# yuliangguo/OmniFusion

Hardware: AMD Instinct MI355X
Metric: panoramas/sec at 512x1024 ERP, N=18 256^2 patches; equi2pers+pers2equi GB/s vs HBM peak (higher is better)
Workload: dtype f16x3 (fp16 hi/lo pairs, fp32 accumulate: fp32-class); 1 GPU; cfg2/cfg4 shard: 8 panoramas/GPU/step, 512x1024 ERP, fov 80, nrows 4 (18 patches); full single-pass spherical_fusion forward (confidence=True) at patch size 128 — the only size the reference network exists at (SURVEY 0.1); random-init weights (seed 42); inputs resident in HBM; resample pair at 18x256^2 reported in roofline_resample; per_gpu_batch=8, global_batch=8, parallelism=image-sharded x1, execution=3 forwards in flight per GPU on 3 streams (spherical_fusion.pipelined)

## Files before the change

omnifusion_amd/csrc/omni_conv_sh.hip:

```cpp
#include "omni_conv_sh_common.h"

namespace {

__constant__ float wino_coef[16][4] = {
    {1, 0, 0, 0}, {1, 1, 0, 0}, {1, -1, 0, 0}, {0, -1, 0, 0},
    {1, 0, 1, 0}, {1, 1, 1, 1}, {1, -1, 1, -1}, {0, -1, 0, -1},
    {1, 0, -1, 0}, {1, 1, -1, -1}, {1, -1, -1, 1}, {0, -1, 0, 1},
    {0, 0, -1, 0}, {0, 0, -1, -1}, {0, 0, -1, 1}, {0, 0, 0, 1}};
template <int BM, int BN, int WM, int WN, int NST = 3, int NL = 0, bool PP = false, bool WINO = false, bool X1 = false>
__global__ __launch_bounds__(64 * (WM * WN + NL)) void conv_sh_kernel(ShConvArgs a)
{
    static_assert(!(WINO && X1), "Winograd: f16x3 only");
    static_assert(!PP || (NL > 0 && WM * WN == 8 && NST >= 3), "ping-pong: eight matrix waves (two per SIMD) + loader waves, three stages");
    static_assert(!WINO || (PP && BM / WM == 32 && BN / WN == 32), "Winograd: the ping-pong kernel with 32 x 32 wave tiles");
    constexpr int NW = WM * WN, LW = NL > 0 ? NL : NW, RPP = 8 * LW;
    constexpr int TM = BM / WM / 32, TN = BN / WN / 32;
    constexpr int APASS = BM / RPP, BPASS = BN / RPP, LPS = APASS + BPASS;
    static_assert(APASS >= 1 && BPASS >= 1, "a tile side must cover at least one DMA pass");
    constexpr int A_BYTES = BM * 128, STAGE = (BM + BN) * 128;
    __shared__ __attribute__((aligned(1024))) unsigned char lds[NST * STAGE];
    __shared__ long long cst[OMNI_ABL(32768) ? 256 : 1];
    const bool stamped = OMNI_ABL(32768) && blockIdx.x == 0 && blockIdx.y == 0 && a.ws != nullptr && a.splitk <= 1;
    auto cstamp = [&](int k) { if (OMNI_ABL(32768) && stamped && (threadIdx.x & 63) == 0 && k < 256) cst[k] = clock64(); };
    auto cdump = [&]() { if (OMNI_ABL(32768) && stamped && threadIdx.x == 0) for (int i = 0; i < 256; ++i) reinterpret_cast<long long*>(a.ws)[i] = cst[i]; };
// ... 477 lines not shown

template <bool X1, int BM, int BN, int WM, int WN, int NST = 3, int NL = 0>
void launch_sh(ShConvArgs a, hipStream_t s)
{
    const int tiles = ((a.rows + BM - 1) / BM) * (a.Cout / BN);
    if constexpr (NL > 0 && WM * WN == 8) {
        if (omni_options().conv_pingpong) {
            hipLaunchKernelGGL((conv_sh_kernel<BM, BN, WM, WN, NST, NL, true, false, X1>), dim3(tiles, a.splitk > 1 ? a.splitk : 1), dim3(64 * (WM * WN + NL)), 0, s, a);
            return;
        }
    }
    hipLaunchKernelGGL((conv_sh_kernel<BM, BN, WM, WN, NST, NL, false, false, X1>), dim3(tiles, a.splitk > 1 ? a.splitk : 1), dim3(64 * (WM * WN + NL)), 0, s, a);
}

}

static int conv2d_sh_impl(const void* src1, const void* src2, const void* wt16, const float* bias,
                          const void* res, void* dst, int fmt, int M, int H, int W, int C1, int C2, int Cout,
                          int KH, int KW, int stride, int pad, int act, int splitk, float* ws, size_t ws_bytes,
                          const float* post, size_t post_elems, omni_stream_t stream, bool reduce = true);
extern "C" int omni_conv2d_sh_f16x3_ws(const void* src1, const void* src2, const void* wt16, const float* bias,
                                       const void* res, void* dst, int fmt, int M, int H, int W, int C1, int C2, int Cout,
                                       int KH, int KW, int stride, int pad, int act, int splitk, float* ws, size_t ws_bytes,
                                       omni_stream_t stream)
{
    return conv2d_sh_impl(src1, src2, wt16, bias, res, dst, fmt, M, H, W, C1, C2, Cout, KH, KW, stride, pad, act, splitk, ws, ws_bytes,
                          nullptr, 0, stream);
}
extern "C" int omni_conv2d_sh_f16x3_post_ws(const void* src1, const void* src2, const void* wt16, const float* bias,
                                            const void* res, void* dst, int fmt, int M, int H, int W, int C1, int C2, int Cout,
                                            int KH, int KW, int stride, int pad, int act, int splitk, float* ws, size_t ws_bytes,
                                            const float* post, size_t post_elems, omni_stream_t stream)
{
    return conv2d_sh_impl(src1, src2, wt16, bias, res, dst, fmt, M, H, W, C1, C2, Cout, KH, KW, stride, pad, act, splitk, ws, ws_bytes,
                          post, post_elems, stream);
}
extern "C" int omni_gemm_sh_f16x3_ln512_ws(const void* x, const void* wt16, const float* bias, const float* res, float* tok, const float* ln_g, const float* ln_b,
                                           float eps, void* y, int fmt, int rows, int K, int splitk, float* ws, size_t ws_bytes, omni_stream_t stream)
{
    if (!x || !wt16 || !tok || !ln_g || !ln_b || !y) OMNI_FAIL(OMNI_ERR_INVALID, "omni_gemm_sh_f16x3_ln512: null pointer");
    if (rows <= 0 || K <= 0 || K % 32) OMNI_FAIL(OMNI_ERR_INVALID, "omni_gemm_sh_f16x3_ln512: bad shape");
    if (fmt & 8) OMNI_FAIL(OMNI_ERR_UNSUPPORTED, "omni_gemm_sh_f16x3_ln512: no f16x1 form (fmt bit 3)");
    const int S = std::min(splitk, K / 32);
    if (S < 2) OMNI_FAIL(OMNI_ERR_INVALID, "omni_gemm_sh_f16x3_ln512: needs a split-K plan (splitk >= 2); an unsplit GEMM writes its result in its own epilogue");
    const int rc = conv2d_sh_impl(x, nullptr, wt16, bias, res, tok, 2, rows, 1, 1, K, 0, 512, 1, 1, 1, 0, OMNI_ACT_NONE, S, ws, ws_bytes, nullptr, 0, stream, false);
    if (rc != OMNI_OK) return rc;
    hipStream_t s = (hipStream_t)stream;
    if (fmt & 1) hipLaunchKernelGGL(sh_splitk_reduce_ln512_kernel<true>, dim3((rows + 3) / 4), dim3(256), 0, s, (const float*)ws, bias, res, tok, ln_g, ln_b, y, rows, S, (size_t)rows * 512, eps);
    else         hipLaunchKernelGGL(sh_splitk_reduce_ln512_kernel<false>, dim3((rows + 3) / 4), dim3(256), 0, s, (const float*)ws, bias, res, tok, ln_g, ln_b, y, rows, S, (size_t)rows * 512, eps);
    OMNI_HIP(hipGetLastError());
    return OMNI_OK;
}

template <bool X1>
static void conv_sh_select(const ShConvArgs& a, int fmt, hipStream_t s)
{
    const int KH = a.KH, KW = a.KW, stride = a.stride, pad = a.pad, H = a.H, W = a.W, M = a.M, Cout = a.Cout;
    const int ksteps = KH * KW * ((a.C1 + a.C2) / 32);
    const long long rows = a.rows;
    if (a.splitk <= 1 && KH == 3 && KW == 3 && stride == 1 && pad == 1 && H == W && (W == 16 || (W == 8 && omni_options().conv_img >= 2)) && rows % 128 == 0 &&
        Cout % 64 == 0 && !(fmt & 4) && omni_options().conv_img > 0 && !omni_options().conv_nohalo) {
        const int grid = (int)(rows / 128) * (Cout / 64);
        if (omni_options().conv_halo_bn == 32) {
            if (W == 16) omni_halo_launch(&a, 32, 4, false, 16, X1, 2 * grid, s);
            else         omni_halo_launch(&a, 32, 4, false, 8, X1, 2 * grid, s);
        }
        else if (W == 16) omni_halo_launch(&a, 64, 4, false, 16, X1, grid, s);
        else         omni_halo_launch(&a, 64, 4, false, 8, X1, grid, s);
        return;
    }
    if (a.splitk <= 1 && KH == 3 && KW == 3 && stride == 1 && pad == 1 && W % HT_W == 0 && H % 4 == 0 && !omni_options().conv_nohalo) {
        const int th = (H % 8 == 0 && omni_options().conv_halo_th == 8) ? 8 : 4;
        const int grid = M * (H / th) * (W / HT_W);
        if (th == 8) {
            if (Cout % 64 == 0 && omni_options().conv_halo_bn != 32) omni_halo_launch(&a, 64, 8, false, 0, X1, grid * (Cout / 64), s);
            else                omni_halo_launch(&a, 32, 8, false, 0, X1, grid * (Cout / 32), s);
        } else {
            const bool bn32 = omni_options().conv_halo_bn == 32 || ((fmt & 4) && omni_options().conv_halo_bn_lat == 32);
            if (Cout % 64 == 0 && !bn32) omni_halo_launch(&a, 64, 4, false, 0, X1, grid * (Cout / 64), s);
            else                omni_halo_launch(&a, 32, 4, false, 0, X1, grid * (Cout / 32), s);
        }
        return;
    }
    int tile = omni_options().conv_sh_tile;
    if (tile < 0) tile = 8;
    const int pm = omni_options().conv_pm;
    const bool pm_shape = pm > 0 && KH == 3 && KW == 3 && stride == 1 && pad == 1 && H == W && (W == 8 || W == 4) && Cout % 64 == 0 && !a.post &&
                          omni_options().conv_pingpong && !(pm == 3 && W != 8) && !(pm == 4 && W != 4);
    if (pm_shape && pm == 2) { omni_conv_pm_launch(&a, Cout % 128 == 0 ? 128 : 64, X1, s); return; }
    const bool big256 = tile == 8 && Cout % 128 == 0 && ((rows + 255) / 256) * (long long)(Cout / 128) * a.splitk >= std::max(1, omni_options().conv_big_blocks);
    if (pm_shape && tile == 8 && !big256) {
        if (Cout % 128 == 0 && ((rows + 127) / 128) * (long long)(Cout / 128) * a.splitk >= 128) { omni_conv_pm_launch(&a, 128, X1, s); return; }
        if (((rows + 127) / 128) * (long long)(Cout / 64) * a.splitk >= 128) { omni_conv_pm_launch(&a, 64, X1, s); return; }
    }
    if (Cout % 64 != 0) launch_sh<X1, 128, 32, 4, 1>(a, s);
    else if (tile == 2 && Cout % 128 == 0) launch_sh<X1, 128, 128, 2, 2>(a, s);
    else if (tile == 1) launch_sh<X1, 128, 64, 2, 2>(a, s);
    else if (tile == 3) launch_sh<X1, 128, 64, 4, 2>(a, s);
    else if (tile == 4 && Cout % 128 == 0) launch_sh<X1, 128, 128, 4, 2>(a, s);
    else if (tile == 8 && Cout % 128 == 0 && ((rows + 255) / 256) * (long long)(Cout / 128) * a.splitk >= std::max(1, omni_options().conv_big_blocks)) launch_sh<X1, 256, 128, 4, 2>(a, s);
    else if (tile == 8 && Cout % 128 == 0 && ((rows + 127) / 128) * (long long)(Cout / 128) * a.splitk >= 128) launch_sh<X1, 128, 128, 4, 2, 3, 4>(a, s);
    else if (tile == 8 && ((rows + 127) / 128) * (long long)(Cout / 64) * a.splitk >= 128) launch_sh<X1, 128, 64, 4, 2, 3, 4>(a, s);
    else if (tile == 9 && Cout % 128 == 0 && ((rows + 255) / 256) * (long long)(Cout / 128) * a.splitk >= 128) launch_sh<X1, 256, 128, 4, 2>(a, s);
    else if (tile == 9 && Cout % 128 == 0 && ((rows + 127) / 128) * (long long)(Cout / 128) * a.splitk >= 128) launch_sh<X1, 128, 128, 4, 2>(a, s);
    else if (tile == 9 && ((rows + 127) / 128) * (long long)(Cout / 64) * a.splitk >= 128) launch_sh<X1, 128, 64, 4, 2>(a, s);
    else if (tile >= 5 && tile <= 7 && Cout % 128 == 0 && ((rows + 127) / 128) * (long long)(Cout / 128) * a.splitk >= (32ll << (tile - 4))) launch_sh<X1, 128, 128, 4, 2>(a, s);
    else if (tile >= 5 && tile <= 7 && ((rows + 127) / 128) * (long long)(Cout / 64) * a.splitk >= (32ll << (tile - 4))) launch_sh<X1, 128, 64, 4, 2>(a, s);
    else if (((rows + 63) / 64) * (long long)(Cout / 64) * a.splitk <= 256 && ksteps >= 8 && !omni_options().conv_nodeep) {
        if (omni_options().conv_deep_loaders) launch_sh<X1, 64, 64, 2, 2, 6, 4>(a, s);
        else launch_sh<X1, 64, 64, 2, 2, 6>(a, s);
    }
    else launch_sh<X1, 64, 64, 2, 2>(a, s);
// ... 22 lines not shown
    const long long rows = (long long)M * a.Ho * a.Wo;
    if (rows <= 0 || rows >= (1ll << 31) || (long long)M * H * W >= (1ll << 31))
        OMNI_FAIL(OMNI_ERR_UNSUPPORTED, "omni_conv2d_sh: too many pixels for 32-bit row indices");
    a.rows = (int)rows;
    const int ksteps = KH * KW * ((C1 + C2) / 32);
    if ((long long)M * H * W * (C1 > C2 ? C1 : C2) * 4 >= (1ll << 31) || (long long)Cout * ksteps * 128 >= (1ll << 31))
        OMNI_FAIL(OMNI_ERR_UNSUPPORTED, "omni_conv2d_sh: an operand of 2 GiB or more (32-bit buffer offsets)");
    int S = splitk;
    if (S > ksteps) S = ksteps;
    if (S > 1 && (!ws || ws_bytes < (size_t)S * rows * Cout * sizeof(float)))
        OMNI_FAIL(OMNI_ERR_INVALID, "omni_conv2d_sh: split-K workspace too small");
    a.splitk = S > 1 ? S : 1; a.ws = ws;
    a.wt_major = omni_options().conv_wt_major == 2 || (omni_options().conv_wt_major == 1 &&
                 (long long)Cout * ksteps * 128 > (long long)M * H * W * (C1 + C2) * 4) ? 1 : 0;
    a.post = post; a.post_rows = 1; a.wino_th = a.wino_tw = a.wino_pix = 0;
    if (post) {
        if (Cout <= 0 || post_elems == 0 || post_elems % (size_t)Cout || post_elems / (size_t)Cout > 0x7fffffffull)
            OMNI_FAIL(OMNI_ERR_INVALID, "omni_conv2d_sh: the post-activation addend must hold whole rows of Cout channels");
        if (a.splitk > 1) OMNI_FAIL(OMNI_ERR_UNSUPPORTED, "omni_conv2d_sh: no post-activation addend with split-K");
        a.post_rows = (unsigned)(post_elems / (size_t)Cout);
    }
    hipStream_t s = (hipStream_t)stream;
    if (fmt & 8) conv_sh_select<true>(a, fmt, s);
    else         conv_sh_select<false>(a, fmt, s);
    OMNI_HIP(hipGetLastError());
    if (a.splitk > 1 && reduce) {
        const size_t n4 = (size_t)rows * Cout / 4;
        hipLaunchKernelGGL(sh_splitk_reduce_kernel, dim3((unsigned)((n4 + 255) / 256)), dim3(256), 0, s, (const float*)ws, bias, res, dst,
                           n4, Cout, a.splitk, (size_t)rows * Cout, act, a.dst_sh, a.res_f32);
        OMNI_HIP(hipGetLastError());
    }
    return OMNI_OK;
}

extern "C" int omni_splitk_reduce_ln512(const float* parts, int nparts, const float* bias, const float* res, float* tok, const float* lg, const float* lb,
                                        float eps, void* y, int fmt, int rows, omni_stream_t stream)
{
    if (!parts || nparts < 1 || !tok || !lg || !lb || !y || rows <= 0) OMNI_FAIL(OMNI_ERR_INVALID, "omni_splitk_reduce_ln512: null pointer or empty input");
    hipStream_t s = (hipStream_t)stream;
    if (fmt & 1) hipLaunchKernelGGL(sh_splitk_reduce_ln512_kernel<true>, dim3((rows + 3) / 4), dim3(256), 0, s, parts, bias, res, tok, lg, lb, y, rows, nparts, (size_t)rows * 512, eps);
    else         hipLaunchKernelGGL(sh_splitk_reduce_ln512_kernel<false>, dim3((rows + 3) / 4), dim3(256), 0, s, parts, bias, res, tok, lg, lb, y, rows, nparts, (size_t)rows * 512, eps);
    OMNI_HIP(hipGetLastError());
    return OMNI_OK;
}

OMNI_SH_OVERFLOW_ACCESSOR(omni_sh_overflow_conv)

extern "C" int omni_sh_overflow(int* flag, int reset)
{
    if (!flag) OMNI_FAIL(OMNI_ERR_INVALID, "omni_sh_overflow: null output");
    OMNI_HIP(hipDeviceSynchronize());
    unsigned v = 0;
    if (omni_sh_overflow_conv(&v, reset) != 0 || omni_sh_overflow_halo(&v, reset) != 0 || omni_sh_overflow_up2(&v, reset) != 0 ||
        omni_sh_overflow_rows(&v, reset) != 0 || omni_sh_overflow_net(&v, reset) != 0 || omni_sh_overflow_pm(&v, reset) != 0)
        OMNI_FAIL(OMNI_ERR_HIP, "omni_sh_overflow: could not read the device flag");
    *flag = v ? 1 : 0;
    return OMNI_OK;
}

extern "C" int omni_sh_from_f32(const float* src, void* dst, size_t n, omni_stream_t stream)
{
    if (!src || !dst || n % 32) OMNI_FAIL(OMNI_ERR_INVALID, "omni_sh_from_f32: null pointer or n % 32 != 0");
    if (n == 0) return OMNI_OK;
    hipLaunchKernelGGL(sh_from_f32_kernel, dim3((unsigned)((n / 4 + 255) / 256)), dim3(256), 0, (hipStream_t)stream, src, dst, n / 4);
    OMNI_HIP(hipGetLastError());
    return OMNI_OK;
}
extern "C" int omni_sh_to_f32(const void* src, float* dst, size_t n, omni_stream_t stream)
{
    if (!src || !dst || n % 32) OMNI_FAIL(OMNI_ERR_INVALID, "omni_sh_to_f32: null pointer or n % 32 != 0");
    if (n == 0) return OMNI_OK;
    hipLaunchKernelGGL(sh_to_f32_kernel, dim3((unsigned)((n / 4 + 255) / 256)), dim3(256), 0, (hipStream_t)stream, src, dst, n / 4);
    OMNI_HIP(hipGetLastError());
    return OMNI_OK;
}

namespace {

__global__ __launch_bounds__(256) void wino_input_sh_kernel(const void* __restrict__ src, void* __restrict__ V, int M, int H, int W, int C, size_t nt)
{
    const size_t i = (size_t)blockIdx.x * 256 + threadIdx.x;
    const int cq = C >> 2;
    if (i >= nt * cq) return;
    const size_t tl = i / cq;
    const int c = (int)(i - tl * cq) * 4;
    const int tw = W >> 1, th = H >> 1;
    const int m = (int)(tl / (size_t)(th * tw)), rem = (int)(tl - (size_t)m * th * tw), ty = rem / tw, tx = rem - ty * tw;
    f4v d[4][4];
#pragma unroll
    for (int a_ = 0; a_ < 4; ++a_)
#pragma unroll
        for (int b_ = 0; b_ < 4; ++b_) {
            const int y = 2 * ty - 1 + a_, x = 2 * tx - 1 + b_;
            d[a_][b_] = ((unsigned)y < (unsigned)H && (unsigned)x < (unsigned)W) ? act_load4<true>(src, (((size_t)m * H + y) * W + x) * C + c) : (f4v)(0.0f);
        }
    f4v u[4][4];
#pragma unroll
    for (int b_ = 0; b_ < 4; ++b_) { u[0][b_] = d[0][b_] - d[2][b_]; u[1][b_] = d[1][b_] + d[2][b_]; u[2][b_] = d[2][b_] - d[1][b_]; u[3][b_] = d[1][b_] - d[3][b_]; }
#pragma unroll
    for (int xi = 0; xi < 4; ++xi) {
        const f4v v0 = u[xi][0] - u[xi][2], v1 = u[xi][1] + u[xi][2], v2 = u[xi][2] - u[xi][1], v3 = u[xi][1] - u[xi][3];
        act_store4<true>(V, ((size_t)(4 * xi + 0) * nt + tl) * C + c, v0);
        act_store4<true>(V, ((size_t)(4 * xi + 1) * nt + tl) * C + c, v1);
        act_store4<true>(V, ((size_t)(4 * xi + 2) * nt + tl) * C + c, v2);
        act_store4<true>(V, ((size_t)(4 * xi + 3) * nt + tl) * C + c, v3);
    }
}
// ... 43 lines not shown
```

omnifusion_amd/csrc/omni_conv_sh_common.h:

```cpp
#pragma once
#include <stdlib.h>
#include <algorithm>
#include <type_traits>
#include "omni_internal.h"
#include "omni_sh.h"

#ifndef OMNI_CONV_ABL
#define OMNI_CONV_ABL 0
#endif
#define OMNI_ABL(bit) ((OMNI_CONV_ABL & (bit)) != 0)
#ifndef OMNI_PP_PRIO
#define OMNI_PP_PRIO 0
#endif
#ifndef OMNI_G1_PW
#define OMNI_G1_PW 4
#endif

namespace {

typedef float f16v __attribute__((ext_vector_type(16)));
typedef float f4v __attribute__((ext_vector_type(4)));
typedef _Float16 h8v __attribute__((ext_vector_type(8)));
typedef _Float16 h4v __attribute__((ext_vector_type(4)));
typedef _Float16 h2v __attribute__((ext_vector_type(2)));
// ... 149 lines not shown
            if (a.res) {
#pragma unroll
                for (int e = 0; e < 4; ++e) { v0[e] += fmaf((float)rl[kk][e], 4.8828125e-4f, (float)rh[kk][e]); v1[e] += fmaf((float)rl[kk][4 + e], 4.8828125e-4f, (float)rh[kk][4 + e]); }
            }
            if (a.act == OMNI_ACT_RELU) {
#pragma unroll
                for (int e = 0; e < 4; ++e) { v0[e] = fmaxf(v0[e], 0.f); v1[e] = fmaxf(v1[e], 0.f); }
            } else if (a.act == OMNI_ACT_GELU) {
#pragma unroll
                for (int e = 0; e < 4; ++e) { v0[e] = 0.5f * v0[e] * (1.0f + erff(v0[e] * 0.70710678118654752440f)); v1[e] = 0.5f * v1[e] * (1.0f + erff(v1[e] * 0.70710678118654752440f)); }
            }
            if (post) { v0 += pa[kk]; v1 += pb[kk]; }
            h4v h0, l0, h1, l1;
            sh_split4(v0, h0, l0); sh_split4(v1, h1, l1);
            h8v oh, ol;
#pragma unroll
            for (int e = 0; e < 4; ++e) { oh[e] = h0[e]; oh[4 + e] = h1[e]; ol[e] = l0[e]; ol[4 + e] = l1[e]; }
            *reinterpret_cast<h8v*>((unsigned char*)a.dst + off[kk]) = oh;
            *reinterpret_cast<h8v*>((unsigned char*)a.dst + off[kk] + 64) = ol;
        }
    }
}

__device__ __forceinline__ void splitk_finish(f4v v, size_t o, const float* __restrict__ bias, const void* __restrict__ res, void* __restrict__ dst,
                                              int Cout, int act, int dst_sh, int res_f32)
{
    if (bias) v += *reinterpret_cast<const f4v*>(bias + (o % Cout));
    if (res && res_f32) v += *reinterpret_cast<const f4v*>((const float*)res + o);
    else if (res) {
        const unsigned char* rp = (const unsigned char*)res + sh_off(o);
        v += sh_join4(*reinterpret_cast<const h4v*>(rp), *reinterpret_cast<const h4v*>(rp + 64));
    }
    if (act == OMNI_ACT_RELU) { v.x = fmaxf(v.x, 0.f); v.y = fmaxf(v.y, 0.f); v.z = fmaxf(v.z, 0.f); v.w = fmaxf(v.w, 0.f); }
    else if (act == OMNI_ACT_GELU) {
#pragma unroll
        for (int e = 0; e < 4; ++e) v[e] = 0.5f * v[e] * (1.0f + erff(v[e] * 0.70710678118654752440f));
    }
    if (dst_sh) {
        h4v hi, lo; sh_split4(v, hi, lo);
        unsigned char* dp = (unsigned char*)dst + sh_off(o);
        *reinterpret_cast<h4v*>(dp) = hi; *reinterpret_cast<h4v*>(dp + 64) = lo;
    } else {
        *reinterpret_cast<f4v*>((float*)dst + o) = v;
    }
}

constexpr int HT_W = 32, HPW = HT_W + 2;

}

void omni_halo_launch(const void* args, int bn, int th, bool up2, int iw, bool x1, unsigned grid, hipStream_t s);
void omni_conv_pm_launch(const void* args, int bn, bool x1, hipStream_t s);
int omni_sh_overflow_pm(unsigned* out, int reset);
int omni_sh_overflow_halo(unsigned* out, int reset);
int omni_sh_overflow_up2(unsigned* out, int reset);
int omni_sh_overflow_rows(unsigned* out, int reset);
int omni_sh_overflow_net(unsigned* out, int reset);
```

omnifusion_amd/csrc/omni_geometry.hip:

```cpp
#include <math.h>
#include <stdlib.h>
#include <string.h>
#include <mutex>
#include <vector>
#include <memory>

#include "omni_internal.h"

static thread_local std::string g_err;
void omni_set_error(const std::string& msg) { g_err = msg; }
extern "C" const char* omni_last_error(void) { return g_err.c_str(); }
extern "C" int omni_version(void) { return OMNI_VERSION; }

namespace {
struct OptName { const char* name; const char* env; int OmniOptions::* field; int dflt; };
const OptName kOpts[] = {
    {"conv_sh_tile", "OMNI_CONV_SH_TILE", &OmniOptions::conv_sh_tile, -1},
    {"conv_nohalo", "OMNI_CONV_NOHALO", &OmniOptions::conv_nohalo, 0},
    {"conv_halo_th", "OMNI_CONV_HALO_TH", &OmniOptions::conv_halo_th, 4},
    {"conv_big_blocks", "OMNI_CONV_BIG_BLOCKS", &OmniOptions::conv_big_blocks, 128},
    {"conv_halo_bn_lat", "OMNI_CONV_HALO_BN_LAT", &OmniOptions::conv_halo_bn_lat, 32},
    {"conv_deep_loaders", "OMNI_CONV_DEEP_LOADERS", &OmniOptions::conv_deep_loaders, 1},
    {"conv_halo_up2_bn_lat", "OMNI_CONV_HALO_UP2_BN_LAT", &OmniOptions::conv_halo_up2_bn_lat, 64},
    {"conv_halo_bn", "OMNI_CONV_HALO_BN", &OmniOptions::conv_halo_bn, 64},
    {"conv_img", "OMNI_CONV_IMG", &OmniOptions::conv_img, 1},
    {"conv_nodeep", "OMNI_CONV_NODEEP", &OmniOptions::conv_nodeep, 0},
    {"conv_pingpong", "OMNI_CONV_PINGPONG", &OmniOptions::conv_pingpong, 1},
    {"conv_pm", "OMNI_CONV_PM", &OmniOptions::conv_pm, 1},
    {"conv_noxcd", "OMNI_CONV_NOXCD", &OmniOptions::conv_noxcd, 0},
    {"conv_wt_major", "OMNI_CONV_WT_MAJOR", &OmniOptions::conv_wt_major, 1},
    {"conv_stem_pc", "OMNI_CONV_STEM_PC", &OmniOptions::conv_stem_pc, 1},
    {"conv_epi_lds", "OMNI_CONV_EPI_LDS", &OmniOptions::conv_epi_lds, 1},
    {"conv_up2_persist", "OMNI_CONV_UP2_PERSIST", &OmniOptions::conv_up2_persist, 1},
    {"splitk_max", "OMNI_SPLITK_MAX", &OmniOptions::splitk_max, 0},
    {"e2p_gather", "OMNI_E2P_GATHER", &OmniOptions::e2p_gather, 0},
    {"e2p_notab", "OMNI_E2P_NOTAB", &OmniOptions::e2p_notab, 0},
    {"e2p_verbose", "OMNI_E2P_VERBOSE", &OmniOptions::e2p_verbose, 0},
    {"e2p_bwd_simple", "OMNI_E2P_BWD_SIMPLE", &OmniOptions::e2p_bwd_simple, 0},
    {"p2e_bwd_simple", "OMNI_P2E_BWD_SIMPLE", &OmniOptions::p2e_bwd_simple, 0},
    {"bwd_table_mb", "OMNI_BWD_TABLE_MB", &OmniOptions::bwd_table_mb, 1024},
    {"bwd_wide", "OMNI_BWD_WIDE", &OmniOptions::bwd_wide, 1},
    {"bwd_lmax", "OMNI_BWD_LMAX", &OmniOptions::bwd_lmax, 0},
    {"bwd_chunk", "OMNI_BWD_CHUNK", &OmniOptions::bwd_chunk, 0},
    {"p2e_gather", "OMNI_P2E_GATHER", &OmniOptions::p2e_gather, 0},
    {"e2p_nbuf", "OMNI_E2P_NBUF", &OmniOptions::e2p_nbuf, 0},
    {"e2p_slot_kb", "OMNI_E2P_SLOT_KB", &OmniOptions::e2p_slot_kb, 6},
    {"e2p_tile_h", "OMNI_E2P_TILE_H", &OmniOptions::e2p_tile_h, 0},
    {"e2p_ref_lds", "OMNI_E2P_REF_LDS", &OmniOptions::e2p_ref_lds, 1},
    {"e2p_store", "OMNI_E2P_STORE", &OmniOptions::e2p_store, 1},
    {"e2p_slots", "OMNI_E2P_SLOTS", &OmniOptions::e2p_slots, 0},
    {"e2p_split", "OMNI_E2P_SPLIT", &OmniOptions::e2p_split, 0},
    {"e2p_full", "OMNI_E2P_FULL", &OmniOptions::e2p_full, -1},
    {"e2p_fb_planes", "OMNI_E2P_FB_PLANES", &OmniOptions::e2p_fb_planes, 0},
    {"e2p_fb_pos", "OMNI_E2P_FB_POS", &OmniOptions::e2p_fb_pos, 0},
    {"e2p_region", "OMNI_E2P_REGION", &OmniOptions::e2p_region, 0},
    {"p2e_band", "OMNI_P2E_BAND", &OmniOptions::p2e_band, 0},
    {"p2e_nbuf", "OMNI_P2E_NBUF", &OmniOptions::p2e_nbuf, 0},
    {"p2e_lds_kb", "OMNI_P2E_LDS_KB", &OmniOptions::p2e_lds_kb, 0},
    {"p2e_planes", "OMNI_P2E_PLANES", &OmniOptions::p2e_planes, 0},
    {"p2e_walk", "OMNI_P2E_WALK", &OmniOptions::p2e_walk, 1},
    {"p2e_tile8", "OMNI_P2E_TILE8", &OmniOptions::p2e_tile8, 1},
    {"p2e_store", "OMNI_P2E_STORE", &OmniOptions::p2e_store, 1},
    {"fv_bwd_lds", "OMNI_FV_BWD_LDS", &OmniOptions::fv_bwd_lds, 1},
    {"geom_cache_max", "OMNI_GEOM_CACHE_MAX", &OmniOptions::geom_cache_max, 16},
    {"chamfer_split", "OMNI_CHAMFER_SPLIT", &OmniOptions::chamfer_split, 1},
    {"augment_lut", "OMNI_AUGMENT_LUT", &OmniOptions::augment_lut, 1},
    {"conv_wgrad_rows", "OMNI_CONV_WGRAD_ROWS", &OmniOptions::conv_wgrad_rows, 0},
};
}

OmniOptions& omni_options()
{
    static OmniOptions o = [] {
        OmniOptions v;
        for (const OptName& k : kOpts) {
            const char* e = getenv(k.env);
            v.*(k.field) = e ? (*e ? atoi(e) : 1) : k.dflt;
        }
        return v;
    }();
    return o;
}

int omni_num_cus()
{
    static int cus[64] = {0};
    int dev = 0;
    if (hipGetDevice(&dev) != hipSuccess || dev < 0 || dev >= 64) return 256;
    if (cus[dev] == 0) {
        int n = 0;
        cus[dev] = (hipDeviceGetAttribute(&n, hipDeviceAttributeMultiprocessorCount, dev) == hipSuccess && n > 0) ? n : 256;
    }
    return cus[dev];
}

extern "C" int omni_set_option(const char* name, int value)
{
    if (!name) OMNI_FAIL(OMNI_ERR_INVALID, "omni_set_option: null name");
    for (const OptName& k : kOpts)
        if (strcmp(k.name, name) == 0) { omni_options().*(k.field) = value; return OMNI_OK; }
    OMNI_FAIL(OMNI_ERR_INVALID, std::string("omni_set_option: unknown option '") + name + "'");
}

extern "C" int omni_get_option(const char* name, int* value)
{
    if (!name || !value) OMNI_FAIL(OMNI_ERR_INVALID, "omni_get_option: null argument");
    for (const OptName& k : kOpts)
        if (strcmp(k.name, name) == 0) { *value = omni_options().*(k.field); return OMNI_OK; }
    OMNI_FAIL(OMNI_ERR_INVALID, std::string("omni_get_option: unknown option '") + name + "'");
}

#ifdef OMNI_DEBUG_BUILD
int omni_debug_bits(const char* env_name) { const char* d = getenv(env_name); return d ? atoi(d) : 0; }
static long long* g_omni_trace = nullptr;
long long* omni_debug_trace_buf() { return g_omni_trace; }
extern "C" int omni_debug_set_trace(long long* buf) { g_omni_trace = buf; return OMNI_OK; }
#endif

namespace {
// ... 216 lines not shown
```

omnifusion_amd/csrc/omni_internal.h:

```cpp
#pragma once
#include <mutex>
#include <hip/hip_runtime.h>
#include <hip/hip_fp16.h>
#include <stdint.h>
#include <string>
#include <vector>

#include "../../include/omnifusion.h"

#define OMNI_MAX_PATCH 46
#define OMNI_WAVE 64

void omni_set_error(const std::string& msg);
#define OMNI_FAIL(code, msg) do { omni_set_error(msg); return (code); } while (0)
#define OMNI_HIP(expr) do { hipError_t e_ = (expr); if (e_ != hipSuccess) {                   \
        omni_set_error(std::string(#expr) + ": " + hipGetErrorString(e_)); return OMNI_ERR_HIP; } } while (0)

struct OmniOptions {
    int conv_sh_tile;
    int conv_nohalo;
    int conv_halo_th;
    int conv_halo_bn_lat;
    int conv_halo_up2_bn_lat;
    int conv_deep_loaders;
    int conv_big_blocks;
    int conv_halo_bn;
    int conv_img;
    int conv_nodeep;
    int conv_pingpong;
    int conv_pm;
    int conv_noxcd;
    int conv_wt_major;
    int conv_stem_pc;
    int conv_epi_lds;
    int conv_up2_persist;
    int splitk_max;
    int e2p_gather;
    int e2p_notab;
    int e2p_verbose;
    int e2p_bwd_simple;
    int p2e_bwd_simple;
    int p2e_gather;
    int e2p_nbuf;
    int e2p_store;
    int e2p_slots;
    int e2p_split;
    int e2p_full;
    int e2p_fb_planes;
    int e2p_region;
    int e2p_fb_pos;
    int e2p_ref_lds;
    int e2p_tile_h;
    int e2p_slot_kb;
    int p2e_band;
    int p2e_lds_kb;
    int p2e_nbuf;
    int p2e_planes;
    int p2e_store;
    int p2e_tile8;
    int p2e_walk;
    int bwd_wide;
    int bwd_chunk;
    int bwd_lmax;
    int bwd_table_mb;
    int fv_bwd_lds;
    int geom_cache_max;
    int chamfer_split;
    int augment_lut;
    int conv_wgrad_rows;
};
OmniOptions& omni_options();
int omni_num_cus();

#ifdef OMNI_DEBUG_BUILD
#define OMNI_DBG(a, bit) (((a).dbg & (bit)) != 0)
int omni_debug_bits(const char* env_name);
long long* omni_debug_trace_buf();
#else
#define OMNI_DBG(a, bit) false
#endif

struct PatchTab {
    int   N;
    float lam0[OMNI_MAX_PATCH];
    float slam[OMNI_MAX_PATCH];
    float clam[OMNI_MAX_PATCH];
    float sphi[OMNI_MAX_PATCH];
    float cphi[OMNI_MAX_PATCH];
};

constexpr int OMNI_SP_LMAX = 48;
struct OmniSpTable {
    uint2* ent = nullptr; int* slice_off = nullptr; int* cnt = nullptr;
    uint2* long_ent = nullptr; int* long_off = nullptr; int* long_row = nullptr;
    int nrows = 0, nslices = 0, nlong = 0, ok = 0;
    long long nent = 0, npadded = 0, nlong_ent = 0;
};
void omni_sp_free(OmniSpTable& t);
struct omni_geometry;
int omni_bwd_workspace(omni_geometry* g, hipStream_t stream, size_t bytes, float** out);

struct omni_geometry {
    int device;
    int pinned;
    int nrows, N;
    float fov_h, fov_w;
    int ph, pw, H, W;
    PatchTab e2p;
    PatchTab p2e;
    float center_p[2 * OMNI_MAX_PATCH];
    float2* row_trig;
    float2* col_trig;
    unsigned long long* cand;
    int ntx;
    struct P2ETiles { uint2* ent; int max_chunks; int max_cand; int ok; int sum_chunks; uint2* ord; int nslots; unsigned char* walk; int nslots_walk; } p2e_tiles[4];
    int p2e_tx, p2e_ty;
    int4* p2e_bwd_box; float* p2e_rden; int p2e_btx, p2e_bty, p2e_bwd_ok;
    int* p2e_bwd_ids; int p2e_bwd_nsmall, p2e_bwd_nbig;
    struct E2PWorkTab { long long key; uint4* dev; int nblocks; };
    struct E2PTiles { uint2* ent; int* fb; int nfb; int max_chunks; int tw, th, tx, ty; int ok;
                      int* order; int norder;
// ... 60 lines not shown
```

omnifusion_amd/isa.py:

```python
import os
import re
import subprocess
import sys
import tempfile

LLVM = os.environ.get("OMNI_LLVM_BIN", "/opt/rocm/lib/llvm/bin")
TARGET = "hipv4-amdgcn-amd-amdhsa--gfx950"
FORBIDDEN = re.compile(r"\bv_pk_(mul|add|fma)_f32\b")
COUNTED = ("e2p_box_kernel", "p2e_lds_kernel", "p2e_walk_kernel", "e2p_ref_kernel")
HOT = ("conv_sh_kernel", "conv3x3_halo_sh_kernel", "conv3x3_up2_g1_kernel", "stem_f16x3_pc_kernel", "heads_kernel", "maxpool_kernel",
       "layernorm512_kernel", "attention_kernel", "upsample_sh8_kernel")
HOST_ONLY = ("omni_png.o", "omni_geometry.o")


def _device_object(obj, tmp):
    fat = os.path.join(tmp, "fat.bin")
    co = os.path.join(tmp, "dev.co")
    r = subprocess.run([os.path.join(LLVM, "llvm-objcopy"), "--dump-section", f".hip_fatbin={fat}", obj, os.path.join(tmp, "copy.o")],
                       stderr=subprocess.DEVNULL)
    if r.returncode != 0 or not os.path.exists(fat) or os.path.getsize(fat) == 0:
        return None
    subprocess.check_call([os.path.join(LLVM, "clang-offload-bundler"), "--unbundle", "--type=o", f"--input={fat}",
                           f"--targets={TARGET}", f"--output={co}"])
    return co


def disassemble(obj):
    with tempfile.TemporaryDirectory() as tmp:
        co = _device_object(obj, tmp)
        if co is None:
            return ""
        return subprocess.check_output([os.path.join(LLVM, "llvm-objdump"), "-d", "--mcpu=gfx950", co]).decode()


def kernel_meta(obj):
    with tempfile.TemporaryDirectory() as tmp:
        co = _device_object(obj, tmp)
        if co is None:
            return []
        txt = subprocess.check_output([os.path.join(LLVM, "llvm-readelf"), "--notes", co]).decode()
    out, cur = [], None
    keys = {".vgpr_count": "vgpr", ".agpr_count": "agpr", ".sgpr_count": "sgpr", ".group_segment_fixed_size": "lds",
            ".private_segment_fixed_size": "scratch", ".vgpr_spill_count": "vgpr_spill", ".sgpr_spill_count": "sgpr_spill",
            ".name": "name"}
    for line in txt.splitlines():
        m = re.match(r"^  - \.(\w+):\s*(\S+)\s*$", line)
        if m:
            cur = {}
            out.append(cur)
            line = "    ." + m.group(1) + ": " + m.group(2)
        m = re.match(r"^    (\.\w+):\s*(\S+)\s*$", line)
        if m and cur is not None and m.group(1) in keys:
            v = m.group(2)
            cur[keys[m.group(1)]] = v if m.group(1) == ".name" else int(v)
    return [k for k in out if "name" in k]


def demangle(names):
    try:
        p = subprocess.run([os.path.join(LLVM, "llvm-cxxfilt")], input="\n".join(names).encode(), stdout=subprocess.PIPE, check=True)
        return p.stdout.decode().splitlines()
    except Exception:
        return list(names)

# ... 68 lines not shown
```

Measured before the change: 4332 panoramas/s.

## Add halo2 3x3 conv kernel reusing row-shifted A fragments across taps

Adds a new 3x3 conv kernel that stages a halo tile of the input once per channel group and streams weights through a four-slot ring. Each wave computes two output rows and carries the previous row's A fragments in registers, so the ky taps reuse loaded values instead of rereading LDS. It is selected by default (option defaults to 1) when the grid has at least 256 blocks, ahead of the existing halo kernels. Costs are more registers, since it is launch-bounded for two blocks per CU, and a new code path that must match the old epilogue's numerics.

```diff
diff --git a/omnifusion_amd/csrc/omni_conv_halo2.hip b/omnifusion_amd/csrc/omni_conv_halo2.hip
--- /dev/null
+++ b/omnifusion_amd/csrc/omni_conv_halo2.hip
@@ -0,0 +1,207 @@
+#include <stdio.h>
+#include <string.h>
+#include "omni_conv_sh_common.h"
+
+namespace {
+
+template <int IW, bool X1>
+__global__ __launch_bounds__(256, 2) void halo2_sh_kernel(ShConvArgs a)
+{
+    static_assert(IW == 0 || IW == 16, "8 x 32 tiles of wide images, or whole 16 x 16 images");
+    constexpr int BN = 64, TN = 2, NW = 4, RPP = 8 * NW, RING = 4, TROWS = 8;
+    constexpr int HROW = IW > 0 ? IW + 2 : HPW;
+    constexpr int HPX = IW > 0 ? (IW + 2) * (IW + 2) : (TROWS + 2) * HPW, HA_INSTR = (HPX * 8 + 63) / 64, HA_BYTES = HA_INSTR * 1024;
+    constexpr int APASS = (HA_INSTR + NW - 1) / NW, BPASS = BN / RPP, B_BYTES = BN * 128;
+    __shared__ __attribute__((aligned(1024))) unsigned char lds[HA_BYTES + RING * B_BYTES];
+    static_assert(sizeof(lds) <= 80 * 1024, "two blocks per CU");
+
+    const int t = threadIdx.x, lane = t & 63;
+    const int wave = __builtin_amdgcn_readfirstlane(t >> 6);
+    const int ntn = a.Cout / BN, tw = IW > 0 ? 1 : a.W / HT_W, th = IW > 0 ? 1 : a.H / TROWS;
+    int bid = a.noxcd ? blockIdx.x : omni_xcd_remap(blockIdx.x, gridDim.x);
+    const int tile_n = bid % ntn; bid /= ntn;
+    const int tx = bid % tw; bid /= tw;
+    const int ty = bid % th; const int m = bid / th;
+    const int y0 = ty * TROWS, x0 = tx * HT_W, col0 = tile_n * BN;
+    const int G1 = a.C1 >> 5, G = (a.C1 + a.C2) >> 5, ksteps = 9 * G;
+
+    const int gs = (lane & 15) ^ ((4 * wave + (lane >> 4)) & 15);
+    const int rl = 8 * wave + 2 * (lane >> 4) + (gs >> 3), pc16 = (gs & 7) * 16;
+    auto halo_pixel = [&](int p) {
+        const int hy = p / HROW, hx = p - hy * HROW;
+        if constexpr (IW > 0) {
+            const int iy = hy - 1, ix = hx - 1;
+            return (p < HPX && (unsigned)iy < (unsigned)IW && (unsigned)ix < (unsigned)IW) ? (m * IW + iy) * IW + ix : -1;
+        } else {
+            const int iy = y0 - 1 + hy, ix = x0 - 1 + hx;
+            return (p < HPX && (unsigned)iy < (unsigned)a.H && (unsigned)ix < (unsigned)a.W) ? (m * a.H + iy) * a.W + ix : -1;
+        }
+    };
+    int wbase[BPASS];
+#pragma unroll
+    for (int i = 0; i < BPASS; ++i) wbase[i] = (col0 + rl + RPP * i) * ksteps * 128 + pc16;
+    const rsrc_t rs1 = make_rsrc(a.src1, (size_t)a.M * a.H * a.W * a.C1 * 4);
+    const rsrc_t rs2 = make_rsrc(a.src2 ? a.src2 : a.src1, a.src2 ? (size_t)a.M * a.H * a.W * a.C2 * 4 : 0);
+    const rsrc_t rsw = make_rsrc(a.wt, (size_t)a.Cout * ksteps * 128);
+
+    auto issue_a = [&](int g) {
+        const bool first = g < G1;
+        const int cs4 = (first ? a.C1 : a.C2) * 4;
+        const int soff = (first ? g : g - G1) * 128 + pc16;
+        unsigned char* sb = lds + wave * 1024;
+        int rlv = rl;
+        asm volatile("" : "+v"(rlv));
+#pragma unroll
+        for (int i = 0; i < APASS; ++i) {
+            if (wave + NW * i < HA_INSTR) {
+                const int px = halo_pixel(rlv + RPP * i);
+                const int off = px >= 0 ? px * cs4 + soff : (int)0x80000000;
+                if (first) dma16(rs1, sb + i * (1024 * NW), off, 0);
+                else       dma16(rs2, sb + i * (1024 * NW), off, 0);
+            }
+        }
+    };
+    auto issue_b = [&](int g, int tap, int slot) {
+        unsigned char* sb = lds + HA_BYTES + slot * B_BYTES + wave * 1024;
+        const int soff = (tap * G + g) * 128;
+#pragma unroll
+        for (int i = 0; i < BPASS; ++i) dma16(rsw, sb + i * (1024 * NW), wbase[i], soff);
+    };
+
+    int ao[4][3];
+#pragma unroll
+    for (int r = 0; r < 4; ++r)
+#pragma unroll
+        for (int kx = 0; kx < 3; ++kx) {
+            int q;
+            if constexpr (IW > 0) q = (4 * wave + 2 * ((lane & 31) >> 4) + r) * HROW + (lane & 15) + kx;
+            else                  q = (2 * wave + r) * HROW + (lane & 31) + kx;
+            const int d = q >> 1;
+            ao[r][kx] = d * 256 + ((((q & 1) * 8 + (lane >> 5)) ^ (d & 15)) * 16);
+        }
+    int fo[4];
+    {
+        const int r = lane & 31, v = r >> 1, h = lane >> 5;
+#pragma unroll
+        for (int k = 0; k < 4; ++k) fo[k] = v * 256 + ((((r & 1) * 8 + 2 * k + h) ^ v) * 16);
+    }
+
+    f16v acc[2][TN], acc1[2][TN];
+#pragma unroll
+    for (int p = 0; p < 2; ++p)
+#pragma unroll
+        for (int j = 0; j < TN; ++j) { acc[p][j] = (f16v)(0.0f); acc1[p][j] = (f16v)(0.0f); }
+    h8v kh[3][2], kl[3][2];
+
+    issue_a(0);
+    issue_b(0, 0, 0); issue_b(0, 1, 1); issue_b(0, 2, 2);
+    int T = 0;
+    for (int g = 0; g < G; ++g) {
+#pragma unroll
+        for (int tap = 0; tap < 9; ++tap) {
+            const int ky = tap / 3, kx = tap - 3 * ky;
+            if (tap == 0 || T + 1 >= ksteps) wait_vm<0>();
+            else if (T + 2 >= ksteps) wait_vm<BPASS>();
+            else wait_vm<2 * BPASS>();
+            wait_lds_reads();
+            __builtin_amdgcn_s_barrier();
+            asm volatile("" ::: "memory");
+            if (T + 3 < ksteps) {
+                if (tap + 3 < 9) issue_b(g, tap + 3, (T + 3) & 3);
+                else             issue_b(g + 1, tap + 3 - 9, (T + 3) & 3);
+            }
+            const unsigned char* sB = lds + HA_BYTES + (T & 3) * B_BYTES;
+            int a_old = ao[0][kx], a_new = ao[ky + 1][kx];
+            asm volatile("" : "+v"(a_old), "+v"(a_new));
+#pragma unroll
+            for (int kc = 0; kc < 2; ++kc) {
+                if (ky == 0) {
+                    kh[kx][kc] = *reinterpret_cast<const h8v*>(lds + (a_old ^ (kc * 32)));
+                    if constexpr (!X1) kl[kx][kc] = *reinterpret_cast<const h8v*>(lds + (a_old ^ (64 + kc * 32)));
+                }
+                const h8v nh = *reinterpret_cast<const h8v*>(lds + (a_new ^ (kc * 32)));
+                h8v nl;
+                if constexpr (!X1) nl = *reinterpret_cast<const h8v*>(lds + (a_new ^ (64 + kc * 32)));
+#pragma unroll
+                for (int j = 0; j < TN; ++j) {
+                    const unsigned char* bp = sB + j * 32 * 128;
+                    const h8v bh = *reinterpret_cast<const h8v*>(bp + fo[kc]);
+                    h8v bl;
+                    if constexpr (!X1) bl = *reinterpret_cast<const h8v*>(bp + fo[2 + kc]);
+                    acc[0][j] = __builtin_amdgcn_mfma_f32_32x32x16_f16(bh, kh[kx][kc], acc[0][j], 0, 0, 0);
+                    if constexpr (!X1) {
+                        acc1[0][j] = __builtin_amdgcn_mfma_f32_32x32x16_f16(bl, kh[kx][kc], acc1[0][j], 0, 0, 0);
+                        acc1[0][j] = __builtin_amdgcn_mfma_f32_32x32x16_f16(bh, kl[kx][kc], acc1[0][j], 0, 0, 0);
+                    }
+                    acc[1][j] = __builtin_amdgcn_mfma_f32_32x32x16_f16(bh, nh, acc[1][j], 0, 0, 0);
+                    if constexpr (!X1) {
+                        acc1[1][j] = __builtin_amdgcn_mfma_f32_32x32x16_f16(bl, nh, acc1[1][j], 0, 0, 0);
+                        acc1[1][j] = __builtin_amdgcn_mfma_f32_32x32x16_f16(bh, nl, acc1[1][j], 0, 0, 0);
+                    }
+                }
+                kh[kx][kc] = nh;
+                if constexpr (!X1) kl[kx][kc] = nl;
+            }
+            ++T;
+        }
+        if (g + 1 < G) {
+            wait_lds_reads();
+            __builtin_amdgcn_s_barrier();
+            asm volatile("" ::: "memory");
+            issue_a(g + 1);
+        }
+    }
+
+    int c0[TN];
+#pragma unroll
+    for (int j = 0; j < TN; ++j) c0[j] = col0 + j * 32;
+    size_t r0[2], r1[2];
+#pragma unroll
+    for (int p = 0; p < 2; ++p) {
+        if constexpr (IW > 0) { r0[p] = ((size_t)m * IW + 4 * wave + p) * IW; r1[p] = r0[p] + 2 * IW; }
+        else                  { r0[p] = ((size_t)m * a.H + y0 + 2 * wave + p) * a.W + x0; r1[p] = r0[p] + 16; }
+    }
+    if (a.dst_sh && !a.res_f32 && a.epi_lds) {
+        static_assert(NW * 32 * (32 * TN + 4) * 4 <= (int)sizeof(lds), "the transposition tiles must fit the K loop's buffers");
+        wait_lds_reads();
+        __syncthreads();
+        float* tile = reinterpret_cast<float*>(lds) + wave * (32 * (32 * TN + 4));
+#pragma unroll
+        for (int p = 0; p < 2; ++p) {
+            epilogue_tile_lds<TN, true, X1>(acc[p], acc1[p], a, r0[p], 32, c0, lane, tile, r1[p]);
+            asm volatile("s_waitcnt lgkmcnt(0)" ::: "memory");
+        }
+        return;
+    }
+#pragma unroll
+    for (int p = 0; p < 2; ++p) {
+        const size_t r = ((lane & 31) < 16 ? r0[p] : r1[p]) + (lane & 15);
+#pragma unroll
+        for (int j = 0; j < TN; ++j) {
+            const f16v ea[1] = {acc[p][j]}, eb[1] = {acc1[p][j]};
+            const int cj[1] = {c0[j]};
+            epilogue_row<1, 2, X1>(ea, eb, a, r, cj, lane, a.dst_sh != 0);
+        }
+    }
+}
+
+}
+
+OMNI_SH_OVERFLOW_ACCESSOR(omni_sh_overflow_halo2)
+
+void omni_halo2_launch(const void* args, int iw, bool x1, hipStream_t s)
+{
+    ShConvArgs a;
+    memcpy(&a, args, sizeof(a));
+    const bool shape = a.KH == 3 && a.KW == 3 && a.stride == 1 && a.pad == 1 && a.splitk <= 1 && a.Cout % 64 == 0 && a.rows % 256 == 0 &&
+                       (iw == 16 ? (a.H == 16 && a.W == 16) : (iw == 0 && a.W % HT_W == 0 && a.H % 8 == 0));
+    if (!shape) {
+        fprintf(stderr, "omni_halo2_launch: no halo2_sh_kernel<%d> for %d x %d x %d, %d -> %d channels\n", iw, a.M, a.H, a.W, a.C1 + a.C2, a.Cout);
+        abort();
+    }
+    const dim3 grid((unsigned)(a.rows / 256) * (unsigned)(a.Cout / 64)), block(256);
+    if (iw == 16 && !x1) hipLaunchKernelGGL((halo2_sh_kernel<16, false>), grid, block, 0, s, a);
+    else if (iw == 16)   hipLaunchKernelGGL((halo2_sh_kernel<16, true>), grid, block, 0, s, a);
+    else if (!x1)        hipLaunchKernelGGL((halo2_sh_kernel<0, false>), grid, block, 0, s, a);
+    else                 hipLaunchKernelGGL((halo2_sh_kernel<0, true>), grid, block, 0, s, a);
+}
diff --git a/omnifusion_amd/csrc/omni_conv_sh.hip b/omnifusion_amd/csrc/omni_conv_sh.hip
--- a/omnifusion_amd/csrc/omni_conv_sh.hip
+++ b/omnifusion_amd/csrc/omni_conv_sh.hip
@@ -553,12 +553,19 @@
     return OMNI_OK;
 }
 
+constexpr int OMNI_HALO2_MIN_BLOCKS = 256;
 template <bool X1>
 static void conv_sh_select(const ShConvArgs& a, int fmt, hipStream_t s)
 {
     const int KH = a.KH, KW = a.KW, stride = a.stride, pad = a.pad, H = a.H, W = a.W, M = a.M, Cout = a.Cout;
     const int ksteps = KH * KW * ((a.C1 + a.C2) / 32);
     const long long rows = a.rows;
+    if (const int h2 = omni_options().conv_halo2; h2 > 0 && a.splitk <= 1 && KH == 3 && KW == 3 && stride == 1 && pad == 1 && Cout % 64 == 0 && rows % 256 == 0 &&
+        !(fmt & 4) && !omni_options().conv_nohalo && omni_options().conv_halo_bn != 32) {
+        const int iw = (H == 16 && W == 16 && omni_options().conv_img > 0) ? 16 : (W % HT_W == 0 && H % 8 == 0) ? 0 : -1;
+        const long long blocks = (rows / 256) * (Cout / 64);
+        if (iw >= 0 && (h2 == 2 || blocks >= (h2 == 1 ? OMNI_HALO2_MIN_BLOCKS : h2))) { omni_halo2_launch(&a, iw, X1, s); return; }
+    }
     if (a.splitk <= 1 && KH == 3 && KW == 3 && stride == 1 && pad == 1 && H == W && (W == 16 || (W == 8 && omni_options().conv_img >= 2)) && rows % 128 == 0 &&
         Cout % 64 == 0 && !(fmt & 4) && omni_options().conv_img > 0 && !omni_options().conv_nohalo) {
         const int grid = (int)(rows / 128) * (Cout / 64);
@@ -687,7 +694,8 @@
     OMNI_HIP(hipDeviceSynchronize());
     unsigned v = 0;
     if (omni_sh_overflow_conv(&v, reset) != 0 || omni_sh_overflow_halo(&v, reset) != 0 || omni_sh_overflow_up2(&v, reset) != 0 ||
-        omni_sh_overflow_rows(&v, reset) != 0 || omni_sh_overflow_net(&v, reset) != 0 || omni_sh_overflow_pm(&v, reset) != 0)
+        omni_sh_overflow_rows(&v, reset) != 0 || omni_sh_overflow_net(&v, reset) != 0 || omni_sh_overflow_pm(&v, reset) != 0 ||
+        omni_sh_overflow_halo2(&v, reset) != 0)
         OMNI_FAIL(OMNI_ERR_HIP, "omni_sh_overflow: could not read the device flag");
     *flag = v ? 1 : 0;
     return OMNI_OK;
diff --git a/omnifusion_amd/csrc/omni_conv_sh_common.h b/omnifusion_amd/csrc/omni_conv_sh_common.h
--- a/omnifusion_amd/csrc/omni_conv_sh_common.h
+++ b/omnifusion_amd/csrc/omni_conv_sh_common.h
@@ -225,6 +225,8 @@
 void omni_halo_launch(const void* args, int bn, int th, bool up2, int iw, bool x1, unsigned grid, hipStream_t s);
 void omni_conv_pm_launch(const void* args, int bn, bool x1, hipStream_t s);
 int omni_sh_overflow_pm(unsigned* out, int reset);
+void omni_halo2_launch(const void* args, int iw, bool x1, hipStream_t s);
+int omni_sh_overflow_halo2(unsigned* out, int reset);
 int omni_sh_overflow_halo(unsigned* out, int reset);
 int omni_sh_overflow_up2(unsigned* out, int reset);
 int omni_sh_overflow_rows(unsigned* out, int reset);
diff --git a/omnifusion_amd/csrc/omni_geometry.hip b/omnifusion_amd/csrc/omni_geometry.hip
--- a/omnifusion_amd/csrc/omni_geometry.hip
+++ b/omnifusion_amd/csrc/omni_geometry.hip
@@ -65,6 +65,7 @@
     {"geom_cache_max", "OMNI_GEOM_CACHE_MAX", &OmniOptions::geom_cache_max, 16},
     {"chamfer_split", "OMNI_CHAMFER_SPLIT", &OmniOptions::chamfer_split, 1},
     {"augment_lut", "OMNI_AUGMENT_LUT", &OmniOptions::augment_lut, 1},
+    {"conv_halo2", "OMNI_CONV_HALO2", &OmniOptions::conv_halo2, 1},
     {"conv_wgrad_rows", "OMNI_CONV_WGRAD_ROWS", &OmniOptions::conv_wgrad_rows, 0},
 };
 }
diff --git a/omnifusion_amd/csrc/omni_internal.h b/omnifusion_amd/csrc/omni_internal.h
--- a/omnifusion_amd/csrc/omni_internal.h
+++ b/omnifusion_amd/csrc/omni_internal.h
@@ -67,6 +67,7 @@
     int geom_cache_max;
     int chamfer_split;
     int augment_lut;
+    int conv_halo2;
     int conv_wgrad_rows;
 };
 OmniOptions& omni_options();
diff --git a/omnifusion_amd/isa.py b/omnifusion_amd/isa.py
--- a/omnifusion_amd/isa.py
+++ b/omnifusion_amd/isa.py
@@ -9,7 +9,7 @@
 FORBIDDEN = re.compile(r"\bv_pk_(mul|add|fma)_f32\b")
 COUNTED = ("e2p_box_kernel", "p2e_lds_kernel", "p2e_walk_kernel", "e2p_ref_kernel")
 HOT = ("conv_sh_kernel", "conv3x3_halo_sh_kernel", "conv3x3_up2_g1_kernel", "stem_f16x3_pc_kernel", "heads_kernel", "maxpool_kernel",
-       "layernorm512_kernel", "attention_kernel", "upsample_sh8_kernel")
+       "layernorm512_kernel", "attention_kernel", "upsample_sh8_kernel", "halo2_sh_kernel")
 HOST_ONLY = ("omni_png.o", "omni_geometry.o")
 
 
```

Result: faster. 4415 panoramas/s, median of 6 (+1.9%).
